# icameling/lidar_camera_calibration

Measured on AMD Instinct MI355X. Metric: chessboard-corner frames/sec + max corner error (mm), VLP-16 cloud, higher is better.
Workload: dtype f32

## Files before the change

lidar_camera_calibration_amd/csrc/ilcc_api.cpp:

```cpp
#include <hip/hip_runtime.h>

#include <cmath>
#include <cstdio>
#include <cstdlib>
#include <cstring>
#include <fstream>
#include <mutex>
#include <new>
#include <sstream>
#include <string>
#include <vector>

#include "ilcc_internal.h"

using namespace ilcc;

#ifndef ILCC_SLOTS
#define ILCC_SLOTS 4
#endif
constexpr int kSlots = ILCC_SLOTS;
constexpr int kStreams = 3;

enum BatchEvent {
  kEvStart,
// ... 7 lines not shown
  kEvRefined,
  kEvAnchored,
  kEvPrepassed,
  kEvFullStart,
  kEvSearched,
  kEvEnd,
  kEvCount
};
static_assert(kEvCount == ILCC_TIMELINE_COLS - 1, "a timeline row is the slot and one time per event");

struct Slot {
  hipEvent_t ev[kEvCount]{};
  hipEvent_t done = nullptr;
  hipEvent_t late = nullptr;
  hipEvent_t k6_done = nullptr;
  bool allocated = false;
  float4* d_xyzi = nullptr;
  float* d_clicks = nullptr;
  uint64_t* d_off = nullptr;
  ilcc_result* d_res = nullptr;
  float4 *d_roi = nullptr, *d_cluster = nullptr, *d_board = nullptr, *d_pca = nullptr, *d_optim = nullptr;
  float2 *d_yz = nullptr, *d_walk_yz = nullptr;
  uint8_t* d_walk_lab = nullptr;
  uint32_t *d_walk_mi = nullptr, *d_walk_nrim = nullptr;
  uint8_t *d_lab = nullptr, *d_cls = nullptr;
  uint32_t *d_nlab = nullptr, *d_walk = nullptr, *d_counts = nullptr, *d_parent = nullptr, *d_count = nullptr;
  unsigned long long* d_masks = nullptr;
  uint32_t *d_hash_head = nullptr, *d_hash_next = nullptr;
  uint32_t *d_flags = nullptr, *d_nfinite = nullptr, *d_counts_fin = nullptr;
  uint32_t* h_online = nullptr;
// ... 273 lines not shown
  if (need_mask > sl.grp_mask_cap) {
    if (sl.d_grp_mask) (void)hipFree(sl.d_grp_mask);
    sl.d_grp_mask = nullptr;
    sl.grp_mask_cap = 0;
    HIP_TRY(h, hipMalloc((void**)&sl.d_grp_mask, sizeof(uint32_t) * need_mask));
    sl.grp_mask_cap = need_mask;
  }
  return ILCC_OK;
}

int32_t alloc_slot(ilcc_handle* h, Slot& sl) {
  if (sl.allocated) return ILCC_OK;
  const uint64_t np = h->max_points;
  const uint32_t mf = h->max_frames;
  for (auto& ev : sl.ev) HIP_TRY(h, hipEventCreate(&ev));
  HIP_TRY(h, hipEventCreateWithFlags(&sl.done, hipEventDisableTiming));
  HIP_TRY(h, hipEventCreateWithFlags(&sl.late, hipEventDisableTiming));
  HIP_TRY(h, hipEventCreateWithFlags(&sl.k6_done, hipEventDisableTiming));
#define ALLOC(ptr, bytes) HIP_TRY(h, hipMalloc((void**)&(ptr), (size_t)(bytes)))
  ALLOC(sl.d_xyzi, sizeof(float4) * np);
  ALLOC(sl.d_clicks, sizeof(float) * 3 * mf);
  ALLOC(sl.d_off, sizeof(uint64_t) * (mf + 1));
  ALLOC(sl.d_res, sizeof(ilcc_result) * mf);
  ALLOC(sl.d_roi, sizeof(float4) * np);
  ALLOC(sl.d_cluster, sizeof(float4) * np);
  ALLOC(sl.d_board, sizeof(float4) * np);
  ALLOC(sl.d_pca, sizeof(float4) * np);
  ALLOC(sl.d_optim, sizeof(float4) * np);
  ALLOC(sl.d_yz, sizeof(float2) * np);
  ALLOC(sl.d_walk_yz, sizeof(float2) * np);
  ALLOC(sl.d_walk_lab, np);
  ALLOC(sl.d_walk_mi, sizeof(uint32_t) * mf);
  ALLOC(sl.d_walk_nrim, sizeof(uint32_t) * mf);
// ... 228 lines not shown
  g.collect_ties = 1u;
  return g;
}

LocatePlan locate_plan(const ilcc_handle* h, const Slot& sl, const Ctx& c) {
  LocatePlan lp{};
  lp.seed = h->seed_grid;
  lp.map = h->seed_map;
  lp.refine_radius = std::max(1, h->seed_map.stride_th / ILCC_REFINE_RADIUS_DIV);
  lp.sample_min = (uint32_t)ILCC_SEED_POINTS;
  lp.sample_cap = std::max((uint32_t)ILCC_SEED_POINTS, ((c.grid_lds_points >> 3) + 63u) & ~63u);
  lp.out = sl.d_partial4;
  return lp;
}

int32_t enqueue_locate_launches(ilcc_handle* h, Slot& sl, const Ctx& c, hipStream_t s, int32_t refine_radius, GridSeed& located) {
  launch_grid_cost(c, seed_pass(h, sl, c), s, 1, nullptr, true);
  HIP_TRY(h, hipEventRecord(sl.ev[kEvSeeded], s));
  const GridPass refine = refine_pass(h, sl, c, refine_radius);
  launch_grid_cost(c, refine, s, 1, nullptr, true);
  HIP_TRY(h, hipEventRecord(sl.ev[kEvRefined], s));
  located = full_table_records(refine.out, refine.blocks);
  GridPartial* const ping[2] = {sl.d_partial4, sl.d_partial2};
  for (int round = 0; round < kAnchorRounds; ++round) {
    const GridPass anchor = anchor_pass(h, c, located, ping[round & 1]);
    launch_anchor(c, anchor, s);
    located = full_table_records(anchor.out, anchor.blocks);
  }
  return ILCC_OK;
}

int32_t enqueue_grid_search(ilcc_handle* h, Slot& sl, const Ctx& c, hipStream_t s, uint32_t n_frames, bool chain, bool walk_laid_out = false) {
  const bool prune = h->p.grid_prune != 0;
  if (!walk_laid_out) launch_walk_order(c, s);
  HIP_TRY(h, hipEventRecord(sl.ev[kEvWalkOrdered], s));
  GridSeed located{};
  if (h->seed_grid.n_th > 0 && h->p.n_th >= 8 && h->p.n_ty >= 8 && h->p.n_tz >= 8) {
    const LocatePlan lp = locate_plan(h, sl, c);
    const bool fused = n_frames >= (uint32_t)kLocateMinFrames && lp.seed.n_th <= 16 &&
                       locate_lds_bytes(lp.sample_cap, h->grid.n_ty, h->grid.n_tz, lp.seed.n_ty, lp.seed.n_tz) <= 60u * 1024u;
    if (fused) {
      launch_locate(c, s, lp);
      HIP_TRY(h, hipEventRecord(sl.ev[kEvSeeded], s));
      HIP_TRY(h, hipEventRecord(sl.ev[kEvRefined], s));
      located = full_table_records(lp.out, 1);
    } else {
      const int32_t st = enqueue_locate_launches(h, sl, c, s, lp.refine_radius, located);
      if (st != ILCC_OK) return st;
    }
  } else {
    HIP_TRY(h, hipEventRecord(sl.ev[kEvSeeded], s));
    HIP_TRY(h, hipEventRecord(sl.ev[kEvRefined], s));
  }
  HIP_TRY(h, hipEventRecord(sl.ev[kEvAnchored], s));
  GridPass full = full_pass(h, c, located);
  const GroupPrepassPlan gp = group_prepass_plan(h->p);
  full.box_points = gp.box ? (uint32_t)ILCC_BOX_POINTS : 0u;
  if (full.box_points != 0u && gp.on && (size_t)n_frames * gp.groups <= sl.grp_alive_cap &&
      (size_t)n_frames * gp.groups * gp.words <= sl.grp_mask_cap) {
    full.grp_alive = sl.d_grp_alive;
    full.grp_mask = sl.d_grp_mask;
    full.grp_count = gp.groups;
    full.grp_words = gp.words;
    launch_group_prepass(c, full, s);
  } else if (full.box_points != 0u && gp.on) {
    if (h->group_prepass_skipped++ == 0) h->err = "note: k6_group_prepass skipped (mask buffers smaller than this batch needs): slower, results unaffected";
  }
  HIP_TRY(h, hipEventRecord(sl.ev[kEvPrepassed], s));
  const int si = (int)(&sl - h->slots);
  if (chain && h->k6_last >= 0 && h->k6_last != si && h->slots[h->k6_last].busy)
    HIP_TRY(h, hipStreamWaitEvent(s, h->slots[h->k6_last].k6_done, 0));
  HIP_TRY(h, hipEventRecord(sl.ev[kEvFullStart], s));
  launch_grid_cost(c, full, s, 1, nullptr, prune);
  if (chain) {
    HIP_TRY(h, hipEventRecord(sl.k6_done, s));
    h->k6_last = si;
  }
  return ILCC_OK;
}

int32_t enqueue_impl(ilcc_handle* h, int si, hipStream_t s, const float4* d_xyzi, const uint64_t* offsets, uint32_t n_frames,
                     const float* d_clicks, bool front_only, bool no_crop) {
  Slot& sl = h->slots[si];
  uint64_t max_n = 0;
  for (uint32_t f = 0; f < n_frames; ++f) max_n = std::max<uint64_t>(max_n, offsets[f + 1] - offsets[f]);
  uint32_t chunks = (uint32_t)((max_n + kCropChunk - 1) / kCropChunk);
  if (chunks == 0) chunks = 1;
  if ((uint64_t)chunks * n_frames > (uint64_t)h->crop_chunks_cap) {
    h->err = "crop chunk table too small for this (very ragged) batch";
    return ILCC_CAPACITY;
  }
  sl.off.assign(offsets, offsets + n_frames + 1);
  sl.n_frames = n_frames;
  std::memcpy(sl.h_off, sl.off.data(), sizeof(uint64_t) * (n_frames + 1));
  HIP_TRY(h, hipMemcpyAsync(sl.d_off, sl.h_off, sizeof(uint64_t) * (n_frames + 1), hipMemcpyHostToDevice, s));
  Ctx c = make_ctx(h, sl, d_xyzi, d_clicks, n_frames, chunks);
  HIP_TRY(h, hipEventRecord(sl.ev[kEvStart], s));
  if (!no_crop) {
    launch_roi_crop(c, s, sl.ev[kEvCropCounted], !h->separate_launches && n_frames >= (uint32_t)kCropFrameMinFrames);
    HIP_TRY(h, hipEventRecord(sl.ev[kEvCropped], s));
    launch_cluster(c, s);
  } else {
    c.p.cluster_tol = c.p.online_cluster_tol;
    c.wide = 1u;
    Ctx t1 = c;
    t1.online_tier = 1u;
    t1.online_window = 1.25f;
    t1.p.roi_half[0] = t1.p.roi_half[1] = t1.p.roi_half[2] = (double)t1.online_window;
    t1.cluster_bits = cluster_bits_online();
    launch_roi_crop(t1, s, sl.ev[kEvCropCounted]);
    HIP_TRY(h, hipEventRecord(sl.ev[kEvCropped], s));
    launch_cluster(t1, s);
    Ctx t2 = c;
    t2.online_tier = 2u;
    t2.p.roi_half[0] = t2.p.roi_half[1] = t2.p.roi_half[2] = (double)INFINITY;
    launch_roi_crop(t2, s, nullptr);
    launch_cluster(t2, s);
    HIP_TRY(h, hipMemcpyAsync(sl.h_online, sl.d_flags, sizeof(uint32_t) * n_frames, hipMemcpyDeviceToHost, s));
    HIP_TRY(h, hipMemcpyAsync(sl.h_online + h->max_frames, sl.d_nfinite, sizeof(uint32_t) * n_frames, hipMemcpyDeviceToHost, s));
  }
  HIP_TRY(h, hipEventRecord(sl.ev[kEvClustered], s));
  sl.grid = !front_only && h->p.solver == ILCC_SOLVER_GRID;
  const bool one_launch = !h->separate_launches && front_end_fusable(c);
  if (one_launch) {
    launch_front_end(c, s, sl.grid);
    HIP_TRY(h, hipEventRecord(sl.ev[kEvPlane], s));
  } else {
    launch_ransac_plane(c, s);
    HIP_TRY(h, hipEventRecord(sl.ev[kEvPlane], s));
    launch_plane_frame_hist(c, s);
  }
  HIP_TRY(h, hipEventRecord(sl.ev[kEvLabelled], s));
  if (sl.grid) {
    const int32_t st = enqueue_grid_search(h, sl, c, s, n_frames, true, one_launch);
    if (st != ILCC_OK) return st;
  }
  HIP_TRY(h, hipEventRecord(sl.ev[kEvSearched], s));
  if (!front_only) {
    if (sl.grid) {
      launch_pattern_refine_corners(c, s);
    } else {
      launch_refine_corners(c, s);
    }
  }
  HIP_TRY(h, hipEventRecord(sl.ev[kEvEnd], s));
  HIP_TRY(h, hipGetLastError());
  sl.compact = h->result_mode == ILCC_RESULTS_COMPACT;
  sl.rec_corners = board_corners(h->p);
  if (sl.compact) {
    launch_pack_records(sl.d_res, n_frames, sl.rec_corners, 0u, sl.h_rec_dev, s);
  } else {
    HIP_TRY(h, copy_results_trimmed(sl.h_res, sl.d_res, n_frames, sl.rec_corners, s));
  }
  launch_store_to_host(sl.d_iters, sl.h_iters_dev, sizeof(unsigned long long) * kBatchWords, s);
  HIP_TRY(h, hipGetLastError());
  HIP_TRY(h, hipEventRecord(sl.done, s));
  sl.busy = true;
  sl.online = no_crop;
  return ILCC_OK;
}

int32_t run_late(ilcc_handle* h, Slot& sl, hipStream_t s) {
  HIP_TRY(h, hipEventRecord(sl.late, s));
  HIP_TRY(h, hipEventSynchronize(sl.late));
  return ILCC_OK;
}

int32_t ensure_full(ilcc_handle* h, Slot& sl) {
  if (sl.h_res_valid) return ILCC_OK;
  const hipStream_t s = late_stream(h);
  HIP_TRY(h, copy_results_trimmed(sl.h_res, sl.d_res, sl.n_frames, sl.rec_corners, s));
// ... 15 lines not shown
  if (pack_now) launch_pack_records(sl.d_res, n_frames, sl.rec_corners, 0u, sl.h_rec_dev, ls);
  if (d_records || pack_now) {
    const int32_t st = run_late(h, sl, ls);
    if (st != ILCC_OK) return st;
  }
  sl.busy = false;
  sl.h_res_valid = !sl.compact;
  h->last_slot = si;
  if (out) {
    const int32_t st = ensure_full(h, sl);
    if (st != ILCC_OK) return st;
    const size_t row = trimmed_bytes(sl.rec_corners);
    for (uint32_t f = 0; f < n_frames; ++f) std::memcpy(&out[f], &sl.h_res[f], row);
  }
  if (out_compact) std::memcpy(out_compact, sl.h_rec, sizeof(float) * n_frames * rec_w);
  auto span = [&](BatchEvent from, BatchEvent to, float& ms_out) { return hipEventElapsedTime(&ms_out, sl.ev[from], sl.ev[to]); };
  float ms[6];
  HIP_TRY(h, span(kEvStart, kEvCropped, ms[0]));
  HIP_TRY(h, span(kEvCropped, kEvClustered, ms[1]));
  HIP_TRY(h, span(kEvClustered, kEvPlane, ms[2]));
  HIP_TRY(h, span(kEvPlane, kEvLabelled, ms[3]));
  HIP_TRY(h, span(kEvLabelled, kEvSearched, ms[4]));
  HIP_TRY(h, span(kEvSearched, kEvEnd, ms[5]));
  float k6k[6] = {0.f, 0.f, 0.f, 0.f, 0.f, 0.f};
  if (sl.grid) {
    float pre = 0.f;
    HIP_TRY(h, span(kEvLabelled, kEvPrepassed, pre));
    HIP_TRY(h, span(kEvLabelled, kEvWalkOrdered, k6k[0]));
    HIP_TRY(h, span(kEvWalkOrdered, kEvSeeded, k6k[1]));
    HIP_TRY(h, span(kEvSeeded, kEvRefined, k6k[2]));
    HIP_TRY(h, span(kEvRefined, kEvAnchored, k6k[3]));
    HIP_TRY(h, span(kEvAnchored, kEvPrepassed, k6k[4]));
    HIP_TRY(h, span(kEvFullStart, kEvSearched, k6k[5]));
    ms[4] = pre + k6k[5];
  }
  float tot = 0;
  HIP_TRY(h, span(kEvStart, kEvEnd, tot));
  if (h->tl_on && h->tl_ref && sl.grid) {
    h->tl_rows.push_back((double)si);
    for (hipEvent_t e : sl.ev) {
      float t = 0.f;
      HIP_TRY(h, hipEventElapsedTime(&t, h->tl_ref, e));
      h->tl_rows.push_back((double)t);
    }
  }
  ilcc_timing& t = h->timing;
  t.roi_crop = ms[0];
  t.cluster = ms[1];
  t.ransac_plane = ms[2];
  t.plane_frame_hist = ms[3];
  t.grid_cost = ms[4];
  t.refine_corners = ms[5];
  t.total = tot;
  t.batches += 1;
  for (int k = 0; k < 6; ++k) t.stage_ms_sum[k] += ms[k];
// ... 703 lines not shown
  const hipStream_t s = h->stream[take_stream(h)];
  int32_t st = stage_labelled(h, s, yz, label, m);
  if (st != ILCC_OK) return st;
  Slot& sl = h->slots[0];
  uint32_t lds = 1024;
  while (lds < m && lds < (uint32_t)kGridLdsPointsMax) lds <<= 1;
  const uint32_t saved = h->grid_lds_points;
  h->grid_lds_points = std::max(saved, lds);
  const Ctx c = make_ctx(h, sl, nullptr, nullptr, 1, 1);
  h->grid_lds_points = saved;
  const uint32_t inf_bits = 0x7f800000u, zero = 0u;
  HIP_TRY(h, hipMemcpyAsync(sl.d_bound, &inf_bits, sizeof(inf_bits), hipMemcpyHostToDevice, s));
  HIP_TRY(h, hipMemcpyAsync(sl.d_bound_sub, &inf_bits, sizeof(inf_bits), hipMemcpyHostToDevice, s));
  HIP_TRY(h, hipMemcpyAsync(sl.d_tie_count, &zero, sizeof(zero), hipMemcpyHostToDevice, s));
  HIP_TRY(h, hipMemsetAsync(sl.d_iters, 0, sizeof(unsigned long long) * kBatchWords, s));
  st = enqueue_grid_search(h, sl, c, s, 1, false);
  if (st != ILCC_OK) return st;
  launch_pattern_refine_corners(c, s);
  HIP_TRY(h, hipGetLastError());
  SolveRec rec{};
  ilcc_result r;
  HIP_TRY(h, hipMemcpyAsync(&rec, sl.d_solverec, sizeof(rec), hipMemcpyDeviceToHost, s));
  HIP_TRY(h, hipMemcpyAsync(&r, sl.d_res, offsetof(ilcc_result, corners), hipMemcpyDeviceToHost, s));
  {
    const int32_t sst = sync_own(h, s);
    if (sst != ILCC_OK) return sst;
  }
  if (!rec.valid) {
    h->err = "ilcc_grid_solve: the grid search produced no candidate";
    return ILCC_TOO_FEW_POINTS;
// ... 150 lines not shown
```

lidar_camera_calibration_amd/csrc/ilcc_internal.h:

```cpp
#pragma once

#include <hip/hip_runtime.h>
#include <stdint.h>

#include "ilcc_hip.h"

#define ILCC_WAVE 64

namespace ilcc {

constexpr int kCropThreads = 256;
constexpr int kCropChunk = 4096;
#ifndef ILCC_K2_THREADS
#define ILCC_K2_THREADS 256
#endif
constexpr int kFrameThreads = ILCC_K2_THREADS;
#ifndef ILCC_K3_THREADS
#define ILCC_K3_THREADS 256
#endif
#ifndef ILCC_K45_THREADS
#define ILCC_K45_THREADS 256
#endif
constexpr int kPlaneThreads = ILCC_K3_THREADS;
constexpr int kPlaneThreadsSmallBatch = 1024;
// ... 250 lines not shown
constexpr int kLocateMinFrames = 512;

void launch_roi_crop(const Ctx& c, hipStream_t s, hipEvent_t after_count = nullptr, bool one_pass = false);
constexpr int kCropFrameMinFrames = 512;
void launch_cluster(const Ctx& c, hipStream_t s);
void launch_ransac_plane(const Ctx& c, hipStream_t s);
void launch_plane_frame_hist(const Ctx& c, hipStream_t s);
void launch_front_end(const Ctx& c, hipStream_t s, bool walk_layout);
inline bool front_end_fusable(const Ctx& c) {
  return kPlaneThreads == kHistThreads && kHistThreads == kWalkThreads && c.n_frames > (uint32_t)kSmallBatchFrames && !c.wide;
}
void launch_walk_order(const Ctx& c, hipStream_t s);
void launch_grid_cost(const Ctx& c, const GridPass& pass, hipStream_t s, int32_t use_oob, float* cost_volume , bool prune);
void launch_group_prepass(const Ctx& c, const GridPass& full, hipStream_t s);
uint32_t grid_cost_evals_per_count();
void launch_refine_corners(const Ctx& c, hipStream_t s);
void launch_pack_records(const ilcc_result* d_res, uint32_t n_frames, uint32_t n_corners, uint32_t tag_base, float* d_out,
                         hipStream_t s);
void launch_store_to_host(const void* d_src, void* h_dst, size_t bytes, hipStream_t s);
void launch_pattern_refine_corners(const Ctx& c, hipStream_t s);
void launch_pattern_refine_test(const Ctx& c, hipStream_t s, RefineOut* d_io);
hipError_t set_kernel_attributes_k2();
size_t cluster_lds_bytes(uint32_t pts_cap, uint32_t cells_cap, uint32_t bits);
uint32_t cluster_bits_default();
uint32_t cluster_bits_online();
hipError_t set_kernel_attributes_k6();
hipError_t set_kernel_attributes_k7();
void launch_local_solve(const Ctx& c, hipStream_t s, int32_t tlw, int32_t use_oob, double* theta_t,
                        double* cost_iters );

}
```

lidar_camera_calibration_amd/csrc/k7_refine_corners.hip:

```cpp
#include "ilcc_internal.h"

namespace ilcc {

struct Divisor {
  double d, y;
};
__device__ __forceinline__ Divisor make_divisor(double d) { return Divisor{d, 1.0 / d}; }
__device__ __forceinline__ double div_by(double a, const Divisor& v) {
  const double q = a * v.y;
  const double r = __builtin_fma(-q, v.d, a);
  return __builtin_fma(r, v.y, q);
}

struct Board {
  double W, H, g, delta;
};
struct SolveBoard {
  double W, H, delta;
  double Wg2, Hg2;
  Divisor g;
};
__device__ __forceinline__ SolveBoard make_board(const ilcc_params& p) {
  SolveBoard b;
  b.W = (double)p.board_w;
// ... 1082 lines not shown
    out->x[0] = c.p.th_min + (double)st.lat[0] * (c.p.th_step / dv);
    out->x[1] = c.p.ty_min + (double)st.lat[1] * (c.p.ty_step / dv);
    out->x[2] = c.p.tz_min + (double)st.lat[2] * (c.p.tz_step / dv);
    out->cost_a = out->sel = (double)st.cost / kCostQOne;
    out->cost_b = (double)st.alt / kCostQOne;
    out->margin = ((double)st.alt - (double)st.cost) / (double)(st.cost > 0 ? st.cost : 1);
    out->iters_a = st.rounds;
    out->iters_b = st.hops;
    out->phase = st.phase;
    out->valid = 1;
    out->flags = flags | (st.capped ? ILCC_FLAG_REFINE_CAPPED : 0);
    out->ties = (int32_t)n_ties;
  }
}

__global__ __launch_bounds__(kRefineThreadsSmallBatch) void k7r_pattern_refine(Ctx c, SolveRec* rec) {
  extern __shared__ __align__(16) unsigned char smem[];
  __shared__ RefineShared sh;
  const uint32_t f = blockIdx.x;
  if (c.res[f].status != ILCC_OK) {
    if (threadIdx.x == 0) rec[2 * f].valid = 0;
    return;
  }
  float2* s_yz = reinterpret_cast<float2*>(smem);
  uint8_t* s_lab = smem + sizeof(float2) * (size_t)c.grid_lds_points;
  if (c.n_lab[f] <= c.grid_lds_points)
    refine_frame<true>(c, rec, s_yz, s_lab, sh);
  else
    refine_frame<false>(c, rec, s_yz, s_lab, sh);
}

__global__ __launch_bounds__(kRefineThreads) void k7r_pattern_refine_test(Ctx c, RefineOut* io) {
  __shared__ RefineShared sh;
  if (threadIdx.x < kRefineList) sh.acc[0][threadIdx.x] = 0ull;
  __syncthreads();
  const Board bd{(double)c.p.board_w, (double)c.p.board_h, c.p.grid_length, c.p.huber_delta};
  RefineState st;
  st.lat[0] = io->lat[0];
  st.lat[1] = io->lat[1];
  st.lat[2] = io->lat[2];
  st.phase = io->phase;
  st.skip_first = 0;
  int sweep = 0;
  __syncthreads();
  pattern_refine(c, bd, c.yz, c.lab, c.n_lab[0], sh, sweep, st);
  if (threadIdx.x == 0) {
// ... 7 lines not shown
    io->alt_q = st.alt;
  }
}

__device__ __forceinline__ void inv_rigid_apply(const float* T, const float in[3], float out[3]) {
  const float dx = in[0] - T[3], dy = in[1] - T[7], dz = in[2] - T[11];
#pragma unroll
  for (int c = 0; c < 3; ++c) {
    float s = T[0 + c] * dx;
    s = s + T[4 + c] * dy;
    s = s + T[8 + c] * dz;
    out[c] = s;
  }
}

__global__ __launch_bounds__(kSolveThreads) void k7b_corners(Ctx c, const SolveRec* rec, int n_slots) {
  __shared__ float s_T[16];
  __shared__ uint32_t s_hit[kCoverageCellsMax / 32];
  __shared__ uint32_t s_oob;
  const uint32_t f = blockIdx.x;
  ilcc_result* r = &c.res[f];
  if (r->status != ILCC_OK) return;
  const uint32_t tid = threadIdx.x;
  const uint64_t beg = c.off[f];
  SolveRec best = rec[2 * f];
  if (n_slots > 1) {
    const SolveRec o = rec[2 * f + 1];
    if (o.valid && (!best.valid || o.sel < best.sel)) best = o;
  }
  if (!best.valid) {
    if (tid == 0) r->status = ILCC_BAD_ARGUMENT;
    return;
  }
  if (tid == 0) {
    r->theta_t[0] = best.x[0];
// ... 2 lines not shown
    r->cost_a = best.cost_a;
    r->cost_b = best.cost_b;
    r->sel_cost = best.sel;
    r->phase = best.phase;
    r->iters_a = best.iters_a;
    r->iters_b = best.iters_b;
    r->basin_margin = best.margin;
    r->flags = best.flags;
    r->grid_ties = best.ties;
    const float roll = (float)best.x[0];
    const float E = cosf(roll), F = sinf(roll);
    const float T[16] = {1, 0, 0, 0, 0, E, -F, (float)best.x[1], 0, F, E, (float)best.x[2], 0, 0, 0, 1};
    for (int k = 0; k < 16; ++k) s_T[k] = T[k];
    s_oob = 0u;
  }
  for (int k = (int)tid; k < kCoverageCellsMax / 32; k += kSolveThreads) s_hit[k] = 0u;
  __syncthreads();

  const int W = c.p.board_w, H = c.p.board_h;
  {
    const double g = c.p.grid_length, ct = cos(best.x[0]), st = sin(best.x[0]);
    const uint32_t nl = c.n_lab[f];
    const float2* __restrict__ yz = c.yz + beg;
    uint32_t oob = 0;
    for (uint32_t k = tid; k < nl; k += kSolveThreads) {
      const float2 v = yz[k];
      const double yy = ct * (double)v.x - st * (double)v.y + best.x[1];
      const double zz = st * (double)v.x + ct * (double)v.y + best.x[2];
      const double i = (yy + W * g / 2.0) / g, j = (zz + H * g / 2.0) / g;
      if (i > 0.0 && i < (double)W && j > 0.0 && j < (double)H) {
        const int cell = (int)floor(i) * H + (int)floor(j);
        atomicOr(&s_hit[cell >> 5], 1u << (cell & 31));
      } else {
        ++oob;
      }
    }
    if (oob) atomicAdd(&s_oob, oob);
    __syncthreads();
    if (tid == 0) {
      int cells = 0;
      for (int k = 0; k < (W * H + 31) / 32; ++k) cells += __popc(s_hit[k]);
      r->cells_hit = cells;
      r->n_oob = (int32_t)s_oob;
      if (c.p.min_cell_coverage > 0.0 && (double)cells < c.p.min_cell_coverage * (double)(W * H)) r->flags = best.flags | ILCC_FLAG_LOW_COVERAGE;
    }
  }
  const int nc = (W - 1) * (H - 1);
  const int ncc = nc < ILCC_MAX_CORNERS ? nc : ILCC_MAX_CORNERS;
  for (int t = (int)tid; t < ncc; t += kSolveThreads) {
    const int i = 1 + t / (H - 1), j = 1 + t % (H - 1);
    const double xg = (i - (double)W / 2.0) * c.p.grid_length;
    const double yg = (j - (double)H / 2.0) * c.p.grid_length;
    const float pt[3] = {0.0f, (float)xg, (float)yg};
    float a[3], w[3];
    inv_rigid_apply(s_T, pt, a);
    inv_rigid_apply(r->pca, a, w);
    r->corners[3 * t] = w[0];
    r->corners[3 * t + 1] = w[1];
    r->corners[3 * t + 2] = w[2];
  }
  if (tid == 0) r->n_corners = ncc;

  const uint32_t M = (uint32_t)r->n_plane;
  const float4* __restrict__ Q = c.pca + beg;
  float4* __restrict__ O = c.optim + beg;
  for (uint32_t i = tid; i < M; i += kSolveThreads) {
    const float4 v = Q[i];
    float o[3];
#pragma unroll
    for (int rr = 0; rr < 3; ++rr) {
      float s = s_T[4 * rr] * v.x;
      s = s + s_T[4 * rr + 1] * v.y;
      s = s + s_T[4 * rr + 2] * v.z;
      s = s + s_T[4 * rr + 3];
      o[rr] = s;
    }
    O[i] = make_float4(o[0], o[1], o[2], v.w);
  }
  __syncthreads();
  if (tid == 0 && c.p.solver == ILCC_SOLVER_GRID && c.p.ambiguity_eps > 0.0 && best.margin < c.p.ambiguity_eps) r->status = ILCC_AMBIGUOUS;
}

__global__ __launch_bounds__(ILCC_WAVE) void k7_local_solve_test(Ctx c, int tlw, int use_oob, double* theta_t,
                                                                 double* cost_iters) {
  Problem q;
  q.yz = c.yz;
  q.lab = c.lab;
  q.n = c.n_lab[0];
  q.bd = make_board(c.p);
  q.tlw = tlw != 0;
  q.oob = use_oob != 0;
  __shared__ Dog s_dog1;
  double x[3] = {theta_t[0], theta_t[1], theta_t[2]};
  double cost = 0;
  const int it = trust_region_minimize<false>(q, x, cost, c.p.max_iterations, s_dog1);
  if (threadIdx.x == 0) {
    theta_t[0] = x[0];
    theta_t[1] = x[1];
    theta_t[2] = x[2];
    cost_iters[0] = cost;
    cost_iters[1] = (double)it;
  }
}

hipError_t set_kernel_attributes_k7() {
  const int cap = (int)((sizeof(float2) + 1) * (size_t)kGridLdsPointsMax);
  hipError_t e = hipFuncSetAttribute((const void*)k7a_local_solve, hipFuncAttributeMaxDynamicSharedMemorySize, kSolveLdsMax);
  if (e == hipSuccess) e = hipFuncSetAttribute((const void*)k7a_local_solve_wide, hipFuncAttributeMaxDynamicSharedMemorySize, cap);
  if (e == hipSuccess) e = hipFuncSetAttribute((const void*)k7r_pattern_refine, hipFuncAttributeMaxDynamicSharedMemorySize, cap);
  return e;
}

void launch_pattern_refine_corners(const Ctx& c, hipStream_t s) {
  const size_t lds = (sizeof(float2) + 1) * (size_t)c.grid_lds_points;
  const int threads = c.n_frames <= (uint32_t)kSmallBatchFrames ? kRefineThreadsSmallBatch : kRefineThreads;
  hipLaunchKernelGGL(k7r_pattern_refine, dim3(c.n_frames), dim3(threads), lds, s, c, c.solve_rec);
  hipLaunchKernelGGL(k7b_corners, dim3(c.n_frames), dim3(kSolveThreads), 0, s, c, c.solve_rec, 1);
}

void launch_pattern_refine_test(const Ctx& c, hipStream_t s, RefineOut* d_io) {
  hipLaunchKernelGGL(k7r_pattern_refine_test, dim3(1), dim3(kRefineThreads), 0, s, c, d_io);
}

void launch_refine_corners(const Ctx& c, hipStream_t s) {
  const int n_slots = (c.p.solver == ILCC_SOLVER_REFERENCE_LOCAL && c.p.phase_mode == 2) ? 2 : 1;
  if (c.n_frames <= (uint32_t)kSolveWideMaxFrames) {
    const size_t lds1 = (sizeof(float2) + 1) * (size_t)c.grid_lds_points;
    hipLaunchKernelGGL(k7a_local_solve_wide, dim3(c.n_frames, n_slots), dim3(kSolveThreads), lds1, s, c, c.solve_rec);
    hipLaunchKernelGGL(k7b_corners, dim3(c.n_frames), dim3(kSolveThreads), 0, s, c, c.solve_rec, n_slots);
    return;
  }
  Ctx ck = c;
  size_t lds = (sizeof(float2) + 1) * (size_t)c.grid_lds_points * (size_t)(kSolveWaves / n_slots);
  if (lds > (size_t)kSolveLdsMax) {
    ck.grid_lds_points = 0;
    lds = 0;
  }
  const uint32_t solves = c.n_frames * (uint32_t)n_slots;
  hipLaunchKernelGGL(k7a_local_solve, dim3((solves + kSolveWaves - 1) / kSolveWaves), dim3(kSolveThreads), lds, s, ck, c.solve_rec, n_slots);
  hipLaunchKernelGGL(k7b_corners, dim3(c.n_frames), dim3(kSolveThreads), 0, s, c, c.solve_rec, n_slots);
}

void launch_local_solve(const Ctx& c, hipStream_t s, int32_t tlw, int32_t use_oob, double* theta_t,
                        double* cost_iters) {
  hipLaunchKernelGGL(k7_local_solve_test, dim3(1), dim3(ILCC_WAVE), 0, s, c, tlw, use_oob, theta_t, cost_iters);
}

__global__ __launch_bounds__(128) void k9_pack_records(const ilcc_result* __restrict__ res, uint32_t n_corners, uint32_t tag_base,
                                                       float* __restrict__ out) {
  __shared__ uint32_t s_x[2];
  const ilcc_result& r = res[blockIdx.x];
  const uint32_t width = (uint32_t)ILCC_RECORD_HEADER + 3u * n_corners;
  float* o = out + (uint64_t)blockIdx.x * width;
  const uint32_t have = (uint32_t)(r.n_corners < 0 ? 0 : r.n_corners);
  const uint32_t tag = (tag_base + blockIdx.x) & 0xFFFFFFu;
  uint32_t x = 0;
  for (uint32_t k = threadIdx.x; k < width; k += blockDim.x) {
    float v = 0.f;
    if (k >= (uint32_t)ILCC_RECORD_HEADER) {
      const uint32_t c = k - (uint32_t)ILCC_RECORD_HEADER;
      v = (c < 3u * have) ? r.corners[c] : 0.f;
      x ^= __float_as_uint(v) * (2u * c + 1u);
    } else {
      switch (k) {
        case 0: v = (float)r.status; break;
        case 1: v = (float)r.n_corners; break;
        case 2: v = (float)r.phase; break;
        case 3: v = (float)r.grid_index; break;
        case 4: v = (float)r.iters_a; break;
        case 5: v = (float)r.iters_b; break;
        case 6: v = (float)r.cost_a; break;
        case 7: v = (float)r.cost_b; break;
// ... 3 lines not shown
        case 11: v = (float)r.theta_t[2]; break;
        case 12: v = (float)r.n_plane; break;
        case 13: v = (float)r.n_black; break;
        case 14: v = (float)r.n_white; break;
        case 15: v = (float)r.basin_margin; break;
        case 16: v = (float)tag; break;
        case 18: v = (float)r.flags; break;
        case 19: v = (float)r.n_roi; break;
        default: v = 0.f;
      }
    }
    if (k != 17u) o[k] = v;
  }
#pragma unroll
  for (int of = ILCC_WAVE / 2; of > 0; of >>= 1) x ^= __shfl_xor(x, of, ILCC_WAVE);
  if ((threadIdx.x & (ILCC_WAVE - 1)) == 0) s_x[threadIdx.x >> 6] = x;
  __syncthreads();
  if (threadIdx.x == 0) {
    uint32_t t = s_x[0] ^ s_x[1] ^ (tag * 0x9E3779B1u);
    t = (t ^ (t >> 24)) & 0xFFFFFFu;
    o[17] = (float)t;
  }
}

__global__ __launch_bounds__(256) void k_store_to_host(const uint32_t* __restrict__ src, uint32_t* __restrict__ host_dst, uint32_t n_words) {
  for (uint32_t i = blockIdx.x * blockDim.x + threadIdx.x; i < n_words; i += gridDim.x * blockDim.x) host_dst[i] = src[i];
}
void launch_store_to_host(const void* d_src, void* h_dst, size_t bytes, hipStream_t s) {
  const uint32_t n_words = (uint32_t)(bytes / 4);
  if (n_words == 0) return;
  const uint32_t blocks = std::min<uint32_t>(256u, (n_words + 255u) / 256u);
  hipLaunchKernelGGL(k_store_to_host, dim3(blocks), dim3(256), 0, s, static_cast<const uint32_t*>(d_src), static_cast<uint32_t*>(h_dst), n_words);
}

void launch_pack_records(const ilcc_result* d_res, uint32_t n_frames, uint32_t n_corners, uint32_t tag_base, float* d_out,
                         hipStream_t s) {
  if (n_frames) hipLaunchKernelGGL(k9_pack_records, dim3(n_frames), dim3(128), 0, s, d_res, n_corners, tag_base, d_out);
// ... 4 lines not shown
```

Baseline: 1.299 million.

## Fuse refine, corner, record-pack and counter copy into one back-end kernel

The pattern-refine kernel now goes on to compute corners, pack the compact records and copy the iteration counters straight to host memory in the same launch. Previously this took separate corner, pack and store kernels. Timing events are also deduplicated, so an event is recorded only when new work was enqueued since the last one, and adjacent markers share it. This cuts kernel launches and event records per batch, at the cost of more code and extra shared memory in the refine kernel, which may lower occupancy.

Result: no change. 1.311 million, median of 6 (+0.9%).

```diff
diff --git a/lidar_camera_calibration_amd/csrc/ilcc_api.cpp b/lidar_camera_calibration_amd/csrc/ilcc_api.cpp
--- a/lidar_camera_calibration_amd/csrc/ilcc_api.cpp
+++ b/lidar_camera_calibration_amd/csrc/ilcc_api.cpp
@@ -45,6 +45,8 @@
   hipEvent_t done = nullptr;
   hipEvent_t late = nullptr;
   hipEvent_t k6_done = nullptr;
+  hipEvent_t at[kEvCount]{};
+  hipEvent_t tail = nullptr;
   bool allocated = false;
   float4* d_xyzi = nullptr;
   float* d_clicks = nullptr;
@@ -348,9 +350,9 @@
   const uint64_t np = h->max_points;
   const uint32_t mf = h->max_frames;
   for (auto& ev : sl.ev) HIP_TRY(h, hipEventCreate(&ev));
-  HIP_TRY(h, hipEventCreateWithFlags(&sl.done, hipEventDisableTiming));
+  HIP_TRY(h, hipEventCreate(&sl.done));
   HIP_TRY(h, hipEventCreateWithFlags(&sl.late, hipEventDisableTiming));
-  HIP_TRY(h, hipEventCreateWithFlags(&sl.k6_done, hipEventDisableTiming));
+  HIP_TRY(h, hipEventCreate(&sl.k6_done));
 #define ALLOC(ptr, bytes) HIP_TRY(h, hipMalloc((void**)&(ptr), (size_t)(bytes)))
   ALLOC(sl.d_xyzi, sizeof(float4) * np);
   ALLOC(sl.d_clicks, sizeof(float) * 3 * mf);
@@ -609,17 +611,40 @@
   return lp;
 }
 
+inline void enqueued(Slot& sl) { sl.tail = nullptr; }
+int32_t mark(ilcc_handle* h, Slot& sl, BatchEvent e, hipStream_t s) {
+  if (sl.tail == nullptr) {
+    HIP_TRY(h, hipEventRecord(sl.ev[e], s));
+    sl.tail = sl.ev[e];
+  }
+  sl.at[e] = sl.tail;
+  return ILCC_OK;
+}
+int32_t record_own(ilcc_handle* h, Slot& sl, hipEvent_t own, hipStream_t s) {
+  HIP_TRY(h, hipEventRecord(own, s));
+  sl.tail = own;
+  return ILCC_OK;
+}
+#define MARK(h, sl, e, s)                               \
+  do {                                                  \
+    const int32_t mark_st_ = mark((h), (sl), (e), (s)); \
+    if (mark_st_ != ILCC_OK) return mark_st_;           \
+  } while (0)
+
 int32_t enqueue_locate_launches(ilcc_handle* h, Slot& sl, const Ctx& c, hipStream_t s, int32_t refine_radius, GridSeed& located) {
   launch_grid_cost(c, seed_pass(h, sl, c), s, 1, nullptr, true);
-  HIP_TRY(h, hipEventRecord(sl.ev[kEvSeeded], s));
+  enqueued(sl);
+  MARK(h, sl, kEvSeeded, s);
   const GridPass refine = refine_pass(h, sl, c, refine_radius);
   launch_grid_cost(c, refine, s, 1, nullptr, true);
-  HIP_TRY(h, hipEventRecord(sl.ev[kEvRefined], s));
+  enqueued(sl);
+  MARK(h, sl, kEvRefined, s);
   located = full_table_records(refine.out, refine.blocks);
   GridPartial* const ping[2] = {sl.d_partial4, sl.d_partial2};
   for (int round = 0; round < kAnchorRounds; ++round) {
     const GridPass anchor = anchor_pass(h, c, located, ping[round & 1]);
     launch_anchor(c, anchor, s);
+    enqueued(sl);
     located = full_table_records(anchor.out, anchor.blocks);
   }
   return ILCC_OK;
@@ -627,8 +652,11 @@
 
 int32_t enqueue_grid_search(ilcc_handle* h, Slot& sl, const Ctx& c, hipStream_t s, uint32_t n_frames, bool chain, bool walk_laid_out = false) {
   const bool prune = h->p.grid_prune != 0;
-  if (!walk_laid_out) launch_walk_order(c, s);
-  HIP_TRY(h, hipEventRecord(sl.ev[kEvWalkOrdered], s));
+  if (!walk_laid_out) {
+    launch_walk_order(c, s);
+    enqueued(sl);
+  }
+  MARK(h, sl, kEvWalkOrdered, s);
   GridSeed located{};
   if (h->seed_grid.n_th > 0 && h->p.n_th >= 8 && h->p.n_ty >= 8 && h->p.n_tz >= 8) {
     const LocatePlan lp = locate_plan(h, sl, c);
@@ -636,18 +664,19 @@
                        locate_lds_bytes(lp.sample_cap, h->grid.n_ty, h->grid.n_tz, lp.seed.n_ty, lp.seed.n_tz) <= 60u * 1024u;
     if (fused) {
       launch_locate(c, s, lp);
-      HIP_TRY(h, hipEventRecord(sl.ev[kEvSeeded], s));
-      HIP_TRY(h, hipEventRecord(sl.ev[kEvRefined], s));
+      enqueued(sl);
+      MARK(h, sl, kEvSeeded, s);
+      MARK(h, sl, kEvRefined, s);
       located = full_table_records(lp.out, 1);
     } else {
       const int32_t st = enqueue_locate_launches(h, sl, c, s, lp.refine_radius, located);
       if (st != ILCC_OK) return st;
     }
   } else {
-    HIP_TRY(h, hipEventRecord(sl.ev[kEvSeeded], s));
-    HIP_TRY(h, hipEventRecord(sl.ev[kEvRefined], s));
-  }
-  HIP_TRY(h, hipEventRecord(sl.ev[kEvAnchored], s));
+    MARK(h, sl, kEvSeeded, s);
+    MARK(h, sl, kEvRefined, s);
+  }
+  MARK(h, sl, kEvAnchored, s);
   GridPass full = full_pass(h, c, located);
   const GroupPrepassPlan gp = group_prepass_plan(h->p);
   full.box_points = gp.box ? (uint32_t)ILCC_BOX_POINTS : 0u;
@@ -658,17 +687,22 @@
     full.grp_count = gp.groups;
     full.grp_words = gp.words;
     launch_group_prepass(c, full, s);
+    enqueued(sl);
   } else if (full.box_points != 0u && gp.on) {
     if (h->group_prepass_skipped++ == 0) h->err = "note: k6_group_prepass skipped (mask buffers smaller than this batch needs): slower, results unaffected";
   }
-  HIP_TRY(h, hipEventRecord(sl.ev[kEvPrepassed], s));
+  MARK(h, sl, kEvPrepassed, s);
   const int si = (int)(&sl - h->slots);
-  if (chain && h->k6_last >= 0 && h->k6_last != si && h->slots[h->k6_last].busy)
+  if (chain && h->k6_last >= 0 && h->k6_last != si && h->slots[h->k6_last].busy) {
     HIP_TRY(h, hipStreamWaitEvent(s, h->slots[h->k6_last].k6_done, 0));
-  HIP_TRY(h, hipEventRecord(sl.ev[kEvFullStart], s));
+    enqueued(sl);
+  }
+  MARK(h, sl, kEvFullStart, s);
   launch_grid_cost(c, full, s, 1, nullptr, prune);
+  enqueued(sl);
   if (chain) {
-    HIP_TRY(h, hipEventRecord(sl.k6_done, s));
+    const int32_t st = record_own(h, sl, sl.k6_done, s);
+    if (st != ILCC_OK) return st;
     h->k6_last = si;
   }
   return ILCC_OK;
@@ -689,12 +723,20 @@
   sl.n_frames = n_frames;
   std::memcpy(sl.h_off, sl.off.data(), sizeof(uint64_t) * (n_frames + 1));
   HIP_TRY(h, hipMemcpyAsync(sl.d_off, sl.h_off, sizeof(uint64_t) * (n_frames + 1), hipMemcpyHostToDevice, s));
+  enqueued(sl);
   Ctx c = make_ctx(h, sl, d_xyzi, d_clicks, n_frames, chunks);
-  HIP_TRY(h, hipEventRecord(sl.ev[kEvStart], s));
+  MARK(h, sl, kEvStart, s);
   if (!no_crop) {
-    launch_roi_crop(c, s, sl.ev[kEvCropCounted], !h->separate_launches && n_frames >= (uint32_t)kCropFrameMinFrames);
-    HIP_TRY(h, hipEventRecord(sl.ev[kEvCropped], s));
+    const bool one_pass = !h->separate_launches && n_frames >= (uint32_t)kCropFrameMinFrames;
+    launch_roi_crop(c, s, one_pass ? nullptr : sl.ev[kEvCropCounted], one_pass);
+    enqueued(sl);
+    if (one_pass)
+      MARK(h, sl, kEvCropCounted, s);
+    else
+      sl.at[kEvCropCounted] = sl.ev[kEvCropCounted];
+    MARK(h, sl, kEvCropped, s);
     launch_cluster(c, s);
+    enqueued(sl);
   } else {
     c.p.cluster_tol = c.p.online_cluster_tol;
     c.wide = 1u;
@@ -704,7 +746,9 @@
     t1.p.roi_half[0] = t1.p.roi_half[1] = t1.p.roi_half[2] = (double)t1.online_window;
     t1.cluster_bits = cluster_bits_online();
     launch_roi_crop(t1, s, sl.ev[kEvCropCounted]);
-    HIP_TRY(h, hipEventRecord(sl.ev[kEvCropped], s));
+    enqueued(sl);
+    sl.at[kEvCropCounted] = sl.ev[kEvCropCounted];
+    MARK(h, sl, kEvCropped, s);
     launch_cluster(t1, s);
     Ctx t2 = c;
     t2.online_tier = 2u;
@@ -713,43 +757,57 @@
     launch_cluster(t2, s);
     HIP_TRY(h, hipMemcpyAsync(sl.h_online, sl.d_flags, sizeof(uint32_t) * n_frames, hipMemcpyDeviceToHost, s));
     HIP_TRY(h, hipMemcpyAsync(sl.h_online + h->max_frames, sl.d_nfinite, sizeof(uint32_t) * n_frames, hipMemcpyDeviceToHost, s));
-  }
-  HIP_TRY(h, hipEventRecord(sl.ev[kEvClustered], s));
+    enqueued(sl);
+  }
+  MARK(h, sl, kEvClustered, s);
   sl.grid = !front_only && h->p.solver == ILCC_SOLVER_GRID;
   const bool one_launch = !h->separate_launches && front_end_fusable(c);
   if (one_launch) {
     launch_front_end(c, s, sl.grid);
-    HIP_TRY(h, hipEventRecord(sl.ev[kEvPlane], s));
+    enqueued(sl);
+    MARK(h, sl, kEvPlane, s);
   } else {
     launch_ransac_plane(c, s);
-    HIP_TRY(h, hipEventRecord(sl.ev[kEvPlane], s));
+    enqueued(sl);
+    MARK(h, sl, kEvPlane, s);
     launch_plane_frame_hist(c, s);
-  }
-  HIP_TRY(h, hipEventRecord(sl.ev[kEvLabelled], s));
+    enqueued(sl);
+  }
+  MARK(h, sl, kEvLabelled, s);
   if (sl.grid) {
     const int32_t st = enqueue_grid_search(h, sl, c, s, n_frames, true, one_launch);
     if (st != ILCC_OK) return st;
   }
-  HIP_TRY(h, hipEventRecord(sl.ev[kEvSearched], s));
+  MARK(h, sl, kEvSearched, s);
+  sl.compact = h->result_mode == ILCC_RESULTS_COMPACT;
+  sl.rec_corners = board_corners(h->p);
+  const bool one_launch_back = !front_only && !h->separate_launches;
+  const bool packed = one_launch_back && sl.compact;
+  const BackEndOut beo = packed ? BackEndOut{sl.h_rec_dev, sl.rec_corners, sl.h_iters_dev} : BackEndOut{nullptr, 0u, nullptr};
   if (!front_only) {
     if (sl.grid) {
-      launch_pattern_refine_corners(c, s);
+      launch_pattern_refine_corners(c, s, one_launch_back ? &beo : nullptr);
     } else {
-      launch_refine_corners(c, s);
+      launch_refine_corners(c, s, packed ? &beo : nullptr);
     }
-  }
-  HIP_TRY(h, hipEventRecord(sl.ev[kEvEnd], s));
+    enqueued(sl);
+  }
+  if (packed) {
+    const int32_t st = record_own(h, sl, sl.done, s);
+    if (st != ILCC_OK) return st;
+  }
+  MARK(h, sl, kEvEnd, s);
   HIP_TRY(h, hipGetLastError());
-  sl.compact = h->result_mode == ILCC_RESULTS_COMPACT;
-  sl.rec_corners = board_corners(h->p);
-  if (sl.compact) {
-    launch_pack_records(sl.d_res, n_frames, sl.rec_corners, 0u, sl.h_rec_dev, s);
-  } else {
-    HIP_TRY(h, copy_results_trimmed(sl.h_res, sl.d_res, n_frames, sl.rec_corners, s));
-  }
-  launch_store_to_host(sl.d_iters, sl.h_iters_dev, sizeof(unsigned long long) * kBatchWords, s);
-  HIP_TRY(h, hipGetLastError());
-  HIP_TRY(h, hipEventRecord(sl.done, s));
+  if (!packed) {
+    if (sl.compact) {
+      launch_pack_records(sl.d_res, n_frames, sl.rec_corners, 0u, sl.h_rec_dev, s);
+    } else {
+      HIP_TRY(h, copy_results_trimmed(sl.h_res, sl.d_res, n_frames, sl.rec_corners, s));
+    }
+    launch_store_to_host(sl.d_iters, sl.h_iters_dev, sizeof(unsigned long long) * kBatchWords, s);
+    HIP_TRY(h, hipGetLastError());
+    HIP_TRY(h, hipEventRecord(sl.done, s));
+  }
   sl.busy = true;
   sl.online = no_crop;
   return ILCC_OK;
@@ -795,7 +853,10 @@
     for (uint32_t f = 0; f < n_frames; ++f) std::memcpy(&out[f], &sl.h_res[f], row);
   }
   if (out_compact) std::memcpy(out_compact, sl.h_rec, sizeof(float) * n_frames * rec_w);
-  auto span = [&](BatchEvent from, BatchEvent to, float& ms_out) { return hipEventElapsedTime(&ms_out, sl.ev[from], sl.ev[to]); };
+  auto span = [&](BatchEvent from, BatchEvent to, float& ms_out) {
+    ms_out = 0.f;
+    return sl.at[from] == sl.at[to] ? hipSuccess : hipEventElapsedTime(&ms_out, sl.at[from], sl.at[to]);
+  };
   float ms[6];
   HIP_TRY(h, span(kEvStart, kEvCropped, ms[0]));
   HIP_TRY(h, span(kEvCropped, kEvClustered, ms[1]));
@@ -819,7 +880,7 @@
   HIP_TRY(h, span(kEvStart, kEvEnd, tot));
   if (h->tl_on && h->tl_ref && sl.grid) {
     h->tl_rows.push_back((double)si);
-    for (hipEvent_t e : sl.ev) {
+    for (hipEvent_t e : sl.at) {
       float t = 0.f;
       HIP_TRY(h, hipEventElapsedTime(&t, h->tl_ref, e));
       h->tl_rows.push_back((double)t);
@@ -1553,6 +1614,7 @@
   HIP_TRY(h, hipMemcpyAsync(sl.d_bound_sub, &inf_bits, sizeof(inf_bits), hipMemcpyHostToDevice, s));
   HIP_TRY(h, hipMemcpyAsync(sl.d_tie_count, &zero, sizeof(zero), hipMemcpyHostToDevice, s));
   HIP_TRY(h, hipMemsetAsync(sl.d_iters, 0, sizeof(unsigned long long) * kBatchWords, s));
+  enqueued(sl);
   st = enqueue_grid_search(h, sl, c, s, 1, false);
   if (st != ILCC_OK) return st;
   launch_pattern_refine_corners(c, s);
diff --git a/lidar_camera_calibration_amd/csrc/ilcc_internal.h b/lidar_camera_calibration_amd/csrc/ilcc_internal.h
--- a/lidar_camera_calibration_amd/csrc/ilcc_internal.h
+++ b/lidar_camera_calibration_amd/csrc/ilcc_internal.h
@@ -288,11 +288,16 @@
 void launch_grid_cost(const Ctx& c, const GridPass& pass, hipStream_t s, int32_t use_oob, float* cost_volume , bool prune);
 void launch_group_prepass(const Ctx& c, const GridPass& full, hipStream_t s);
 uint32_t grid_cost_evals_per_count();
-void launch_refine_corners(const Ctx& c, hipStream_t s);
+struct BackEndOut {
+  float* records;
+  uint32_t n_corners;
+  unsigned long long* counters;
+};
+void launch_refine_corners(const Ctx& c, hipStream_t s, const BackEndOut* records = nullptr);
 void launch_pack_records(const ilcc_result* d_res, uint32_t n_frames, uint32_t n_corners, uint32_t tag_base, float* d_out,
                          hipStream_t s);
 void launch_store_to_host(const void* d_src, void* h_dst, size_t bytes, hipStream_t s);
-void launch_pattern_refine_corners(const Ctx& c, hipStream_t s);
+void launch_pattern_refine_corners(const Ctx& c, hipStream_t s, const BackEndOut* one_launch = nullptr);
 void launch_pattern_refine_test(const Ctx& c, hipStream_t s, RefineOut* d_io);
 hipError_t set_kernel_attributes_k2();
 size_t cluster_lds_bytes(uint32_t pts_cap, uint32_t cells_cap, uint32_t bits);
diff --git a/lidar_camera_calibration_amd/csrc/k7_refine_corners.hip b/lidar_camera_calibration_amd/csrc/k7_refine_corners.hip
--- a/lidar_camera_calibration_amd/csrc/k7_refine_corners.hip
+++ b/lidar_camera_calibration_amd/csrc/k7_refine_corners.hip
@@ -1120,22 +1120,6 @@
   }
 }
 
-__global__ __launch_bounds__(kRefineThreadsSmallBatch) void k7r_pattern_refine(Ctx c, SolveRec* rec) {
-  extern __shared__ __align__(16) unsigned char smem[];
-  __shared__ RefineShared sh;
-  const uint32_t f = blockIdx.x;
-  if (c.res[f].status != ILCC_OK) {
-    if (threadIdx.x == 0) rec[2 * f].valid = 0;
-    return;
-  }
-  float2* s_yz = reinterpret_cast<float2*>(smem);
-  uint8_t* s_lab = smem + sizeof(float2) * (size_t)c.grid_lds_points;
-  if (c.n_lab[f] <= c.grid_lds_points)
-    refine_frame<true>(c, rec, s_yz, s_lab, sh);
-  else
-    refine_frame<false>(c, rec, s_yz, s_lab, sh);
-}
-
 __global__ __launch_bounds__(kRefineThreads) void k7r_pattern_refine_test(Ctx c, RefineOut* io) {
   __shared__ RefineShared sh;
   if (threadIdx.x < kRefineList) sh.acc[0][threadIdx.x] = 0ull;
@@ -1173,11 +1157,17 @@
   }
 }
 
-__global__ __launch_bounds__(kSolveThreads) void k7b_corners(Ctx c, const SolveRec* rec, int n_slots) {
-  __shared__ float s_T[16];
-  __shared__ uint32_t s_hit[kCoverageCellsMax / 32];
-  __shared__ uint32_t s_oob;
-  const uint32_t f = blockIdx.x;
+struct BackEndShared {
+  float T[16];
+  uint32_t hit[kCoverageCellsMax / 32];
+  uint32_t oob;
+  uint32_t fold[kRefineWavesMax];
+};
+
+__device__ __forceinline__ void corners_frame(const Ctx& c, uint32_t f, const SolveRec* rec, int n_slots, uint32_t nt, BackEndShared& bs) {
+  float* const s_T = bs.T;
+  uint32_t* const s_hit = bs.hit;
+  uint32_t& s_oob = bs.oob;
   ilcc_result* r = &c.res[f];
   if (r->status != ILCC_OK) return;
   const uint32_t tid = threadIdx.x;
@@ -1210,7 +1200,7 @@
     for (int k = 0; k < 16; ++k) s_T[k] = T[k];
     s_oob = 0u;
   }
-  for (int k = (int)tid; k < kCoverageCellsMax / 32; k += kSolveThreads) s_hit[k] = 0u;
+  for (int k = (int)tid; k < kCoverageCellsMax / 32; k += nt) s_hit[k] = 0u;
   __syncthreads();
 
   const int W = c.p.board_w, H = c.p.board_h;
@@ -1219,7 +1209,7 @@
     const uint32_t nl = c.n_lab[f];
     const float2* __restrict__ yz = c.yz + beg;
     uint32_t oob = 0;
-    for (uint32_t k = tid; k < nl; k += kSolveThreads) {
+    for (uint32_t k = tid; k < nl; k += nt) {
       const float2 v = yz[k];
       const double yy = ct * (double)v.x - st * (double)v.y + best.x[1];
       const double zz = st * (double)v.x + ct * (double)v.y + best.x[2];
@@ -1243,7 +1233,7 @@
   }
   const int nc = (W - 1) * (H - 1);
   const int ncc = nc < ILCC_MAX_CORNERS ? nc : ILCC_MAX_CORNERS;
-  for (int t = (int)tid; t < ncc; t += kSolveThreads) {
+  for (int t = (int)tid; t < ncc; t += (int)nt) {
     const int i = 1 + t / (H - 1), j = 1 + t % (H - 1);
     const double xg = (i - (double)W / 2.0) * c.p.grid_length;
     const double yg = (j - (double)H / 2.0) * c.p.grid_length;
@@ -1260,7 +1250,7 @@
   const uint32_t M = (uint32_t)r->n_plane;
   const float4* __restrict__ Q = c.pca + beg;
   float4* __restrict__ O = c.optim + beg;
-  for (uint32_t i = tid; i < M; i += kSolveThreads) {
+  for (uint32_t i = tid; i < M; i += nt) {
     const float4 v = Q[i];
     float o[3];
 #pragma unroll
@@ -1277,81 +1267,20 @@
   if (tid == 0 && c.p.solver == ILCC_SOLVER_GRID && c.p.ambiguity_eps > 0.0 && best.margin < c.p.ambiguity_eps) r->status = ILCC_AMBIGUOUS;
 }
 
-__global__ __launch_bounds__(ILCC_WAVE) void k7_local_solve_test(Ctx c, int tlw, int use_oob, double* theta_t,
-                                                                 double* cost_iters) {
-  Problem q;
-  q.yz = c.yz;
-  q.lab = c.lab;
-  q.n = c.n_lab[0];
-  q.bd = make_board(c.p);
-  q.tlw = tlw != 0;
-  q.oob = use_oob != 0;
-  __shared__ Dog s_dog1;
-  double x[3] = {theta_t[0], theta_t[1], theta_t[2]};
-  double cost = 0;
-  const int it = trust_region_minimize<false>(q, x, cost, c.p.max_iterations, s_dog1);
-  if (threadIdx.x == 0) {
-    theta_t[0] = x[0];
-    theta_t[1] = x[1];
-    theta_t[2] = x[2];
-    cost_iters[0] = cost;
-    cost_iters[1] = (double)it;
-  }
-}
-
-hipError_t set_kernel_attributes_k7() {
-  const int cap = (int)((sizeof(float2) + 1) * (size_t)kGridLdsPointsMax);
-  hipError_t e = hipFuncSetAttribute((const void*)k7a_local_solve, hipFuncAttributeMaxDynamicSharedMemorySize, kSolveLdsMax);
-  if (e == hipSuccess) e = hipFuncSetAttribute((const void*)k7a_local_solve_wide, hipFuncAttributeMaxDynamicSharedMemorySize, cap);
-  if (e == hipSuccess) e = hipFuncSetAttribute((const void*)k7r_pattern_refine, hipFuncAttributeMaxDynamicSharedMemorySize, cap);
-  return e;
-}
-
-void launch_pattern_refine_corners(const Ctx& c, hipStream_t s) {
-  const size_t lds = (sizeof(float2) + 1) * (size_t)c.grid_lds_points;
-  const int threads = c.n_frames <= (uint32_t)kSmallBatchFrames ? kRefineThreadsSmallBatch : kRefineThreads;
-  hipLaunchKernelGGL(k7r_pattern_refine, dim3(c.n_frames), dim3(threads), lds, s, c, c.solve_rec);
-  hipLaunchKernelGGL(k7b_corners, dim3(c.n_frames), dim3(kSolveThreads), 0, s, c, c.solve_rec, 1);
-}
-
-void launch_pattern_refine_test(const Ctx& c, hipStream_t s, RefineOut* d_io) {
-  hipLaunchKernelGGL(k7r_pattern_refine_test, dim3(1), dim3(kRefineThreads), 0, s, c, d_io);
-}
-
-void launch_refine_corners(const Ctx& c, hipStream_t s) {
-  const int n_slots = (c.p.solver == ILCC_SOLVER_REFERENCE_LOCAL && c.p.phase_mode == 2) ? 2 : 1;
-  if (c.n_frames <= (uint32_t)kSolveWideMaxFrames) {
-    const size_t lds1 = (sizeof(float2) + 1) * (size_t)c.grid_lds_points;
-    hipLaunchKernelGGL(k7a_local_solve_wide, dim3(c.n_frames, n_slots), dim3(kSolveThreads), lds1, s, c, c.solve_rec);
-    hipLaunchKernelGGL(k7b_corners, dim3(c.n_frames), dim3(kSolveThreads), 0, s, c, c.solve_rec, n_slots);
-    return;
-  }
-  Ctx ck = c;
-  size_t lds = (sizeof(float2) + 1) * (size_t)c.grid_lds_points * (size_t)(kSolveWaves / n_slots);
-  if (lds > (size_t)kSolveLdsMax) {
-    ck.grid_lds_points = 0;
-    lds = 0;
-  }
-  const uint32_t solves = c.n_frames * (uint32_t)n_slots;
-  hipLaunchKernelGGL(k7a_local_solve, dim3((solves + kSolveWaves - 1) / kSolveWaves), dim3(kSolveThreads), lds, s, ck, c.solve_rec, n_slots);
-  hipLaunchKernelGGL(k7b_corners, dim3(c.n_frames), dim3(kSolveThreads), 0, s, c, c.solve_rec, n_slots);
-}
-
-void launch_local_solve(const Ctx& c, hipStream_t s, int32_t tlw, int32_t use_oob, double* theta_t,
-                        double* cost_iters) {
-  hipLaunchKernelGGL(k7_local_solve_test, dim3(1), dim3(ILCC_WAVE), 0, s, c, tlw, use_oob, theta_t, cost_iters);
-}
-
-__global__ __launch_bounds__(128) void k9_pack_records(const ilcc_result* __restrict__ res, uint32_t n_corners, uint32_t tag_base,
-                                                       float* __restrict__ out) {
-  __shared__ uint32_t s_x[2];
-  const ilcc_result& r = res[blockIdx.x];
+__global__ __launch_bounds__(kSolveThreads) void k7b_corners(Ctx c, const SolveRec* rec, int n_slots) {
+  __shared__ BackEndShared bs;
+  corners_frame(c, blockIdx.x, rec, n_slots, blockDim.x, bs);
+}
+
+__device__ __forceinline__ void pack_frame(const ilcc_result* res, uint32_t f, uint32_t n_corners, uint32_t tag_base, float* out, uint32_t nt,
+                                           BackEndShared& bs) {
+  const ilcc_result& r = res[f];
   const uint32_t width = (uint32_t)ILCC_RECORD_HEADER + 3u * n_corners;
-  float* o = out + (uint64_t)blockIdx.x * width;
+  float* o = out + (uint64_t)f * width;
   const uint32_t have = (uint32_t)(r.n_corners < 0 ? 0 : r.n_corners);
-  const uint32_t tag = (tag_base + blockIdx.x) & 0xFFFFFFu;
+  const uint32_t tag = (tag_base + f) & 0xFFFFFFu;
   uint32_t x = 0;
-  for (uint32_t k = threadIdx.x; k < width; k += blockDim.x) {
+  for (uint32_t k = threadIdx.x; k < width; k += nt) {
     float v = 0.f;
     if (k >= (uint32_t)ILCC_RECORD_HEADER) {
       const uint32_t c = k - (uint32_t)ILCC_RECORD_HEADER;
@@ -1385,13 +1314,134 @@
   }
 #pragma unroll
   for (int of = ILCC_WAVE / 2; of > 0; of >>= 1) x ^= __shfl_xor(x, of, ILCC_WAVE);
-  if ((threadIdx.x & (ILCC_WAVE - 1)) == 0) s_x[threadIdx.x >> 6] = x;
+  if ((threadIdx.x & (ILCC_WAVE - 1)) == 0) bs.fold[threadIdx.x >> 6] = x;
   __syncthreads();
   if (threadIdx.x == 0) {
-    uint32_t t = s_x[0] ^ s_x[1] ^ (tag * 0x9E3779B1u);
+    uint32_t t = tag * 0x9E3779B1u;
+    for (uint32_t w = 0; w < nt / ILCC_WAVE; ++w) t ^= bs.fold[w];
     t = (t ^ (t >> 24)) & 0xFFFFFFu;
     o[17] = (float)t;
   }
+}
+
+__global__ __launch_bounds__(128) void k9_pack_records(const ilcc_result* __restrict__ res, uint32_t n_corners, uint32_t tag_base,
+                                                       float* __restrict__ out) {
+  __shared__ BackEndShared bs;
+  pack_frame(res, blockIdx.x, n_corners, tag_base, out, blockDim.x, bs);
+}
+
+
+__device__ __forceinline__ void corners_records_frame(const Ctx& c, uint32_t f, const SolveRec* rec, int n_slots, const BackEndOut& o,
+                                                      BackEndShared& bs) {
+  const uint32_t nt = blockDim.x;
+  __syncthreads();
+  corners_frame(c, f, rec, n_slots, nt, bs);
+  if (o.records == nullptr) return;
+  __syncthreads();
+  pack_frame(c.res, f, o.n_corners, 0u, o.records, nt, bs);
+  if (f == 0) {
+    const uint32_t* src = reinterpret_cast<const uint32_t*>(c.grid_iters);
+    uint32_t* dst = reinterpret_cast<uint32_t*>(o.counters);
+    for (uint32_t i = threadIdx.x; i < 2u * (uint32_t)kBatchWords; i += nt) dst[i] = src[i];
+  }
+}
+
+__global__ __launch_bounds__(kRefineThreadsSmallBatch) void k7r_pattern_refine(Ctx c, SolveRec* rec, int go_on, BackEndOut o) {
+  extern __shared__ __align__(16) unsigned char smem[];
+  __shared__ RefineShared sh;
+  __shared__ BackEndShared bs;
+  const uint32_t f = blockIdx.x;
+  if (c.res[f].status != ILCC_OK) {
+    if (threadIdx.x == 0) rec[2 * f].valid = 0;
+  } else {
+    float2* s_yz = reinterpret_cast<float2*>(smem);
+    uint8_t* s_lab = smem + sizeof(float2) * (size_t)c.grid_lds_points;
+    if (c.n_lab[f] <= c.grid_lds_points)
+      refine_frame<true>(c, rec, s_yz, s_lab, sh);
+    else
+      refine_frame<false>(c, rec, s_yz, s_lab, sh);
+  }
+  if (go_on) corners_records_frame(c, f, rec, 1, o, bs);
+}
+
+__global__ __launch_bounds__(kSolveThreads) void k7_corners_records(Ctx c, const SolveRec* rec, int n_slots, BackEndOut o) {
+  __shared__ BackEndShared bs;
+  corners_records_frame(c, blockIdx.x, rec, n_slots, o, bs);
+}
+
+__global__ __launch_bounds__(ILCC_WAVE) void k7_local_solve_test(Ctx c, int tlw, int use_oob, double* theta_t,
+                                                                 double* cost_iters) {
+  Problem q;
+  q.yz = c.yz;
+  q.lab = c.lab;
+  q.n = c.n_lab[0];
+  q.bd = make_board(c.p);
+  q.tlw = tlw != 0;
+  q.oob = use_oob != 0;
+  __shared__ Dog s_dog1;
+  double x[3] = {theta_t[0], theta_t[1], theta_t[2]};
+  double cost = 0;
+  const int it = trust_region_minimize<false>(q, x, cost, c.p.max_iterations, s_dog1);
+  if (threadIdx.x == 0) {
+    theta_t[0] = x[0];
+    theta_t[1] = x[1];
+    theta_t[2] = x[2];
+    cost_iters[0] = cost;
+    cost_iters[1] = (double)it;
+  }
+}
+
+hipError_t set_kernel_attributes_k7() {
+  const int cap = (int)((sizeof(float2) + 1) * (size_t)kGridLdsPointsMax);
+  hipError_t e = hipFuncSetAttribute((const void*)k7a_local_solve, hipFuncAttributeMaxDynamicSharedMemorySize, kSolveLdsMax);
+  if (e == hipSuccess) e = hipFuncSetAttribute((const void*)k7a_local_solve_wide, hipFuncAttributeMaxDynamicSharedMemorySize, cap);
+  if (e == hipSuccess) e = hipFuncSetAttribute((const void*)k7r_pattern_refine, hipFuncAttributeMaxDynamicSharedMemorySize, cap);
+  return e;
+}
+
+void launch_pattern_refine_corners(const Ctx& c, hipStream_t s, const BackEndOut* one_launch) {
+  const size_t lds = (sizeof(float2) + 1) * (size_t)c.grid_lds_points;
+  const int threads = c.n_frames <= (uint32_t)kSmallBatchFrames ? kRefineThreadsSmallBatch : kRefineThreads;
+  if (one_launch) {
+    hipLaunchKernelGGL(k7r_pattern_refine, dim3(c.n_frames), dim3(threads), lds, s, c, c.solve_rec, 1, *one_launch);
+    return;
+  }
+  hipLaunchKernelGGL(k7r_pattern_refine, dim3(c.n_frames), dim3(threads), lds, s, c, c.solve_rec, 0, BackEndOut{});
+  hipLaunchKernelGGL(k7b_corners, dim3(c.n_frames), dim3(kSolveThreads), 0, s, c, c.solve_rec, 1);
+}
+
+void launch_pattern_refine_test(const Ctx& c, hipStream_t s, RefineOut* d_io) {
+  hipLaunchKernelGGL(k7r_pattern_refine_test, dim3(1), dim3(kRefineThreads), 0, s, c, d_io);
+}
+
+void launch_refine_corners(const Ctx& c, hipStream_t s, const BackEndOut* records) {
+  const int n_slots = (c.p.solver == ILCC_SOLVER_REFERENCE_LOCAL && c.p.phase_mode == 2) ? 2 : 1;
+  auto corners = [&] {
+    if (records)
+      hipLaunchKernelGGL(k7_corners_records, dim3(c.n_frames), dim3(kSolveThreads), 0, s, c, c.solve_rec, n_slots, *records);
+    else
+      hipLaunchKernelGGL(k7b_corners, dim3(c.n_frames), dim3(kSolveThreads), 0, s, c, c.solve_rec, n_slots);
+  };
+  if (c.n_frames <= (uint32_t)kSolveWideMaxFrames) {
+    const size_t lds1 = (sizeof(float2) + 1) * (size_t)c.grid_lds_points;
+    hipLaunchKernelGGL(k7a_local_solve_wide, dim3(c.n_frames, n_slots), dim3(kSolveThreads), lds1, s, c, c.solve_rec);
+    corners();
+    return;
+  }
+  Ctx ck = c;
+  size_t lds = (sizeof(float2) + 1) * (size_t)c.grid_lds_points * (size_t)(kSolveWaves / n_slots);
+  if (lds > (size_t)kSolveLdsMax) {
+    ck.grid_lds_points = 0;
+    lds = 0;
+  }
+  const uint32_t solves = c.n_frames * (uint32_t)n_slots;
+  hipLaunchKernelGGL(k7a_local_solve, dim3((solves + kSolveWaves - 1) / kSolveWaves), dim3(kSolveThreads), lds, s, ck, c.solve_rec, n_slots);
+  corners();
+}
+
+void launch_local_solve(const Ctx& c, hipStream_t s, int32_t tlw, int32_t use_oob, double* theta_t,
+                        double* cost_iters) {
+  hipLaunchKernelGGL(k7_local_solve_test, dim3(1), dim3(ILCC_WAVE), 0, s, c, tlw, use_oob, theta_t, cost_iters);
 }
 
 __global__ __launch_bounds__(256) void k_store_to_host(const uint32_t* __restrict__ src, uint32_t* __restrict__ host_dst, uint32_t n_words) {
```
